# zwu88/TANTE

Measured on AMD Instinct MI355X. Metric: rollout frames/sec (fwd), TANTE on 256x256 Active Matter, higher is better.
Workload: dtype bf16

## Files before the change

tante_amd/_lib.py:

```python
import ctypes as C
import os

HERE = os.path.dirname(os.path.abspath(__file__))
LIB_PATH = os.environ.get("TANTE_LIB") or os.path.join(HERE, "lib", "libtante_hip.so")

F32, BF16 = 0, 1
ACT_NONE, ACT_GELU_ERF, ACT_GELU_TANH, ACT_RELU = 0, 1, 2, 3
A_LINEAR, A_PATCH_NHWC, A_PATCH_NCHW = 0, 1, 2
E_LINEAR, E_FILM, E_DECONV_NHWC, E_DECONV_NCHW = 0, 1, 2, 3
W_LINEAR, W_CONV_NHWC, W_DECONV_NHWC, W_DECONV_NCHW = 0, 1, 2, 3
W_LINEAR_T, W_CONV_NHWC_T, W_DECONV_NHWC_T, W_DECONV_NCHW_T = 4, 5, 6, 7

c_i32, c_i64, c_f32, c_vp = C.c_int32, C.c_int64, C.c_float, C.c_void_p


class PackGeom(C.Structure):
    _fields_ = [("n_pad", c_i32), ("k_pad", c_i32), ("nt", c_i32), ("cb", c_i32), ("bytes", c_i64)]


class Gemm(C.Structure):
    _fields_ = [
        ("a", c_vp), ("a_dtype", c_i32), ("a_mode", c_i32), ("M", c_i32), ("K", c_i32),
        ("a_s1", c_i64), ("a_s0", c_i64), ("a_off", c_i64), ("a_n0", c_i32),
        ("Hin", c_i32), ("Win", c_i32), ("Cin", c_i32), ("P", c_i32), ("ln", c_i32), ("ln_eps", c_f32),
# ... 195 lines not shown
    "tante_wgrad_multi": ([c_vp, c_vp, c_i32, c_i64, c_i32, c_i32, c_vp, c_vp, c_i32, c_i32, c_i32, c_i32, c_i32, c_i32, c_vp], c_i32),
    "tante_clip_value": ([c_vp, c_i64, c_f32, c_vp], c_i32),
    "tante_rt_reduce_bwd": ([c_vp, c_i32, c_i32, c_vp, c_vp], c_i32),
    "tante_last_error": ([], C.c_char_p),
    "tante_abi_version": ([], c_i32),
    "tante_set_option": ([C.c_char_p, c_i32], c_i32),
    "tante_nan_to_num": ([c_vp, c_vp, c_i64, c_vp], c_i32),
    "tante_head_fused_multi": ([c_i32, c_vp, c_vp, c_vp, c_i32, c_i64, c_i64, c_i64, c_i32, c_i32, c_i32, c_i32, c_i32, c_vp, c_i64, c_vp, c_i64,
                               c_vp], c_i32),
    "tante_head_fused_multi_streams": ([c_i32, c_vp, c_vp, c_vp, c_i32, c_i64, c_i64, c_i64, c_i32, c_i32, c_i32, c_i32, c_i32, c_vp, c_i64, c_vp, c_i64,
                               c_vp], c_i32),
    "tante_spectral_bf16out_supported": ([c_i64, c_i32, c_i32, c_i32, c_i32, c_i32, c_i32], c_i32),
    "tante_spectral_layer_bf16out": ([c_vp, c_i64, c_i32, c_i32, c_i32, c_vp, c_vp, c_i32, c_i32, c_i32, c_i32, c_vp, c_vp, c_i32, c_i32, c_vp, c_vp,
                                     c_i64, c_vp], c_i32),
    "tante_get_option": ([C.c_char_p, c_i32], c_i32),
    "tante_attention_masked": ([c_vp, c_vp, c_i32, c_i32, c_i32, c_i32, c_i32, c_i32, c_vp, c_i64, c_vp, c_vp], c_i32),
    "tante_attention_masked_bwd": ([c_vp, c_vp, c_vp, c_i32, c_i32, c_i32, c_i32, c_i32, c_i32, c_vp, c_i64, c_vp, c_vp, c_vp], c_i32),
    "tante_attention_flash_stats_floats": ([c_i32, C.POINTER(Seq)], c_i64),
    "tante_attention_flash_supported": ([c_i32, c_i32, c_i32, c_i32], c_i32),
    "tante_attention_flash": ([c_vp, c_vp, c_vp, c_i32, c_i32, c_i32, C.POINTER(Seq), c_i32, c_f32, C.c_uint64, c_vp], c_i32),
    "tante_attention_flash_bwd": ([c_vp, c_vp, c_vp, c_vp, c_vp, c_i32, c_i32, c_i32, C.POINTER(Seq), c_i32, c_f32, C.c_uint64, c_vp], c_i32),
    "tante_head_enc_supported": ([c_i32, c_i32], c_i32),
    "tante_head_enc_stream_bytes": ([c_i32], c_i64),
    "tante_head_enc_ws_bytes": ([c_i64], c_i64),
    "tante_pack_head_enc": ([c_vp] * 6 + [c_i32, c_i32, c_vp, c_vp], c_i32),
    "tante_head_enc_fused": ([c_i32, c_vp, c_vp, c_vp, c_i32, c_i64, c_i64, c_i64, c_i32, c_i32, c_i32, c_i32, c_i32, c_vp, c_i64, c_vp, c_i64,
                             c_vp, c_vp, c_vp, c_i64, c_vp], c_i32),
}

LIB_OPTIONS = ("TANTE_ATTN_BWD_HG", "TANTE_ATTN_BWD_NO_SPLIT", "TANTE_ATTN_BWD_VALU", "TANTE_ATTN_FWD_VALU", "TANTE_AXIS_BWD_SMALL_WGS",
               "TANTE_AXIS_BWD_WGS", "TANTE_AXIS_CT", "TANTE_AXIS_FILM", "TANTE_AXIS_GENERIC", "TANTE_AXIS_MFMA", "TANTE_AXIS_NT", "TANTE_AXIS_WGRAD_WGS",
               "TANTE_BLOCK_KERNEL", "TANTE_COLSUM_ROWS", "TANTE_CVIT_CHAIN_TOKENS", "TANTE_ENC23_SPLIT", "TANTE_FILM_BWD_ROWS",
               "TANTE_FS_GROUPS", "TANTE_FS_HALF", "TANTE_FS_SKEW", "TANTE_FS_WAVES", "TANTE_GEMM_NO_LITE", "TANTE_GEMM_SMALLM", "TANTE_GEMM_WGS", "TANTE_HEAD_WAVES",
               "TANTE_IM2COL_TILED", "TANTE_RESIZE_TILED", "TANTE_SPECTRAL_BF16OUT", "TANTE_SPECTRAL_DFT", "TANTE_SPECTRAL_X3", "TANTE_WGRAD_DEEP",
               "TANTE_WGRAD_JOBS", "TANTE_WGRAD_JOBS_WGS", "TANTE_WGRAD_NO_SLAB", "TANTE_WGRAD_NO_TR", "TANTE_WGRAD_REDUCE_NY",
               "TANTE_WGRAD_RG", "TANTE_WGRAD_SLAB_WGS", "TANTE_WGRAD_TR_WGS", "TANTE_WGRAD_WGS", "TANTE_XATTN_GPW", "TANTE_XATTN_VALU",)


_lib = None
ABI_VERSION = 14


def lib():
    global _lib
    if _lib is None:
        if not os.path.exists(LIB_PATH):
            raise RuntimeError(
                f"{LIB_PATH} is missing: build it with `python -m tante_amd.build` "
                "(or __graft_entry__.build()).  tante_amd has no CPU / eager fallback.")
        L = C.CDLL(LIB_PATH)
        for name, (argtypes, restype) in SIGNATURES.items():
            fn = getattr(L, name)
            fn.argtypes = argtypes
            fn.restype = restype
        got = int(L.tante_abi_version())
        if got != ABI_VERSION:
            raise RuntimeError(f"{LIB_PATH}: library ABI {got}, this binding expects {ABI_VERSION} -- a stale build (or a stale variant under "
                               "TANTE_LIB); rebuild with `python -m tante_amd.build`")
        _lib = L
        import warnings
        for k in LIB_OPTIONS:
            v = os.environ.get(k)
            if v is None:
                continue
            try:
                rc = L.tante_set_option(k.encode(), int(v))
            except ValueError:
# ... 20 lines not shown
```

tante_amd/csrc/block_sliced.hip:

```cpp
#include "common.hip.h"
#include "fused_common.hip.h"
#include "fs_common.hip.h"
#include "block_sliced.h"

#if (defined(FS_EXP_NO_SAVE) || defined(FS_EXP_LN_ID) || defined(FS_EXP_GELU_ID) || defined(FS_EXP_NO_RESID) || defined(FS_EXP_NO_STORE) || \
     defined(FS_EXP_TPROP_NO_STORE) || defined(FS_EXP_ROT) || defined(FS_EXP_NO_WLOAD) || defined(FS_EXP_MFMA32)) && !defined(TANTE_ABLATE)
#error "FS_EXP_* timing experiments produce wrong results on purpose: build them with -DTANTE_ABLATE (tools/build_variant.sh), never into the product library"
#endif

namespace {


struct FsArgs {
  float* x;
  const char* w;
  TanteSeq sq;
  int causal;
  float eps;
  int spw;
  unsigned magic;
  float* out;
  unsigned short *xh1, *qkv, *o, *xh2, *hpre, *act;
  float *st1, *x1, *st2;
  float p_drop;
// ... 50 lines not shown
}
__device__ __forceinline__ void tprop_apply(const TpropW& w, f32x4 (&xs)[4]) {
  f32x4 hid[4], yy[4];
#pragma unroll
  for (int e = 0; e < 4; ++e) {
    f32x4 h = w.b1v;
#pragma unroll
    for (int a = 0; a < 4; ++a) h = __builtin_amdgcn_mfma_f32_4x4x1f32(w.w1c[a], xs[a][e], h, 0, 0, 0);
    hid[e] = h;
  }
#pragma unroll
  for (int e = 0; e < 4; ++e) hid[e] = gelu_poly4<false>(hid[e]);
#pragma unroll
  for (int e = 0; e < 4; ++e) {
    f32x4 acc = f32x4{xs[0][e], xs[1][e], xs[2][e], xs[3][e]} + w.b2v;
#pragma unroll
    for (int j = 0; j < 4; ++j) acc = __builtin_amdgcn_mfma_f32_4x4x1f32(w.w2c[j], hid[e][j], acc, 0, 0, 0);
    yy[e] = acc;
  }
#pragma unroll
  for (int t = 0; t < 4; ++t) xs[t] = f32x4{yy[0][t], yy[1][t], yy[2][t], yy[3][t]};
}

constexpr int fs_group(int ntt, int nk) {
  int g = 1;
  for (int d = 1; d <= ntt; ++d)
    if (ntt % d == 0 && d * nk <= 8) g = d;
  return g;
}

template <int TPS, int NTT, int NW, bool TRAIN, int G = 1, bool TPROP = false, bool LASTQ = false>
__global__ __launch_bounds__(64 * NW * G, 2) void block_fs_kernel(FsArgs A) {
  static_assert(!TPROP || (TPS == 1 && !TRAIN), "the fused temporal propagator: T letter (L = 4), inference");
  static_assert(!LASTQ || (TPS == 1 && NW == 4 && G == 1 && !TRAIN), "the last-slot form: T letter (L = 4), 4 waves, inference");
  static_assert(G == 1 || (G == 2 && NW == 4), "the paired form is two 4-wave groups");
  constexpr int RT = 16 / NW;
  constexpr int HPW = RT / 2;
#ifndef FS_PF8
#define FS_PF8 3
#endif
#ifndef FS_PF4
#define FS_PF4 2
#endif
#ifdef FS_NO_TIGHT
  constexpr bool TIGHT = false;
#else
  constexpr bool TIGHT = (NW == 4 && NTT == 4 && (TRAIN || TPS == 0)) || (NW == 8 && NTT == 8);
#endif
  constexpr int PF = (NW == 8 ? FS_PF8 : FS_PF4) - (TIGHT ? 1 : 0);
  constexpr int IMG = 16 * NTT * FS_ROW;
  constexpr int LDS_G = 2 * IMG + 16 * NTT * NW * 8 + FS_BIAS_FLOATS * 4;
  extern __shared__ __attribute__((aligned(16))) char smem_all[];
  const int grp = G == 1 ? 0 : __builtin_amdgcn_readfirstlane((int)threadIdx.x >> 8);
  char* const smem = smem_all + grp * LDS_G;
  char* const bufA = smem;
  char* const bufB = smem + IMG;
  char* const stat = smem + 2 * IMG;
  float* const lbias = (float*)(stat + 16 * NTT * NW * 8);
  const int tid = threadIdx.x & (64 * NW - 1), lane = tid & 63, kk = lane >> 4, l15 = lane & 15;
  const int wave = __builtin_amdgcn_readfirstlane(tid >> 6);
#ifdef FS_XCD_SAMPLE
  const int vblock = (G == 1 && gridDim.x % 8 == 0) ? (int)((blockIdx.x & 7) * (gridDim.x >> 3) + (blockIdx.x >> 3)) : (int)blockIdx.x * G + grp;
#else
  const int vblock = (int)blockIdx.x * G + grp;
#endif
#ifndef FS_SKEW
#define FS_SKEW 1
#endif
  if constexpr (G == 2 && FS_SKEW) {
    if (grp == 1) __builtin_amdgcn_s_barrier();
  }
#ifdef FS_PRIO
  if constexpr (G == 1) {
    if ((__builtin_amdgcn_s_getreg(0x1804) & 1u) == (FS_PRIO & 1)) __builtin_amdgcn_s_setprio(3);
  }
#endif
  if constexpr (!TRAIN && G == 1) {
    if (A.skew > 0 && blockIdx.x >= (gridDim.x >> 1)) {
      for (int i = 0; i < A.skew; ++i) __builtin_amdgcn_s_sleep(8);
    }
  }
  float* const x = A.x;
  const unsigned long long smix = (TRAIN && A.seed_mix) ? *A.seed_mix : 0ull;
  const unsigned long long sd_attn = A.seed_attn ^ smix;
  const int L = A.sq.L;
  const int seq0 = vblock * A.spw;
  const int nlive = min(A.spw, A.sq.nseq - seq0) * L;
  const int nslot = A.spw * L;

  const FsW wq = fs_wstream(A.w, (unsigned)((RT * wave) * FS_FRAG + lane * 16));
  u32x4 wb[PF + 1][RT];
  FS_STAMP(0);
#ifdef TANTE_ABLATE
  if (A.stamps && lane == 0) {
    A.stamps[((long)vblock * 8 + wave) * 20 + 16] = __builtin_amdgcn_s_getreg((31 << 11) | 4);
    A.stamps[((long)vblock * 8 + wave) * 20 + 17] = __builtin_amdgcn_s_getreg((31 << 11) | 20);
    A.stamps[((long)vblock * 8 + wave) * 20 + 18] = __builtin_amdgcn_s_memrealtime();
  }
#endif
  int tslot[2];
  {
    const FsSeqMap smap(A.sq);
#pragma unroll
    for (int h = 0; h < (16 * NTT > 64 ? 2 : 1); ++h) {
      const int slot = lane + 64 * h;
      const int s = (int)(((unsigned)slot * A.magic) >> 16), p = slot - s * L;
      tslot[h] = slot < nlive ? (int)smap.token(A.sq, seq0 + s, p) : -1;
    }
  }
  auto tok_of = [&](int slot) { return __shfl(slot < 64 ? tslot[0] : tslot[16 * NTT > 64 ? 1 : 0], slot & 63); };
  for (int i = tid; i < FS_BIAS_FLOATS / 4; i += 64 * NW) *(f32x4*)(lbias + 4 * i) = *(const f32x4*)((const float*)(A.w + FS_W_BYTES) + 4 * i);
  FS_STAMP(1);
  int tokidx[NTT];
#pragma unroll
  for (int tt = 0; tt < NTT; ++tt) tokidx[tt] = tok_of(16 * tt + l15);

  constexpr int CPR = 4 * RT, RPI = 64 / CPR, ROWB = CPR * 16, TILEB = 16 * ROWB;
  constexpr int NSUB = (IMG / NW) / TILEB >= 2 ? 2 : 1;
  static_assert((IMG / NW) >= TILEB, "staging piece too small");
  char* const stg = bufA + wave * (IMG / NW);
  const int rrow = lane / CPR, rchunk = lane % CPR;
#ifdef FS_TPROP_RECOMPUTE
  auto srow = [&](int j) { return TPROP ? 4 * rrow + j : RPI * j + rrow; };
#else
  auto srow = [&](int j) { return RPI * j + rrow; };
#endif
  auto slice_load = [&](const float* __restrict__ src, f32x4 (&raw)[NTT][RT]) {
#pragma unroll
    for (int tt = 0; tt < NTT; ++tt)
#pragma unroll
      for (int j = 0; j < RT; ++j) {
        const int t = tok_of(16 * tt + srow(j));
        raw[tt][j] = *(const f32x4*)(src + (long)(t < 0 ? 0 : t) * FS_C + 16 * RT * wave + 4 * rchunk);
      }
  };
  auto slice_to_acc = [&](const f32x4 (&raw)[NTT][RT], f32x4 (&acc)[RT][NTT]) {
#pragma unroll
    for (int tt = 0; tt < NTT; ++tt) {
      char* sb = stg + (tt % NSUB) * TILEB;
#pragma unroll
      for (int j = 0; j < RT; ++j) {
        const int r = srow(j);
        *(f32x4*)(sb + r * ROWB + ((rchunk ^ (r & (CPR - 1))) << 4)) = raw[tt][j];
      }
#pragma unroll
      for (int rt = 0; rt < RT; ++rt) acc[rt][tt] = *(const f32x4*)(sb + l15 * ROWB + (((4 * rt + kk) ^ (l15 & (CPR - 1))) << 4));
    }
  };
  constexpr int CPB = 2 * RT, RPB = 64 / CPB;
  const int brow = lane / CPB, bchunk = lane % CPB;
  auto img_rows_store = [&](const char* img, int tt, unsigned short* __restrict__ dst, long dstride, int dcol) {
#pragma unroll
    for (int j = 0; j < 16 / RPB; ++j) {
      const int r = RPB * j + brow, t = tok_of(16 * tt + r);
      const u32x4 v = *(const u32x4*)(img + tt * 8192 + r * FS_ROW + (((CPB * wave + bchunk) ^ r) << 4));
#ifdef FS_EXP_NO_SAVE
      if (t >= 0 && v[0] == 0x12345u) *(u32x4*)(dst + (long)t * dstride + dcol + 16 * RT * wave + 8 * bchunk) = v;
#else
      if (t >= 0) *(u32x4*)(dst + (long)t * dstride + dcol + 16 * RT * wave + 8 * bchunk) = v;
#endif
    }
  };
  auto slice_store = [&](float* __restrict__ dst, const f32x4 (&acc)[RT][NTT]) {
#pragma unroll
    for (int tt = 0; tt < NTT; ++tt) {
      char* sb = stg + (tt % NSUB) * TILEB;
#pragma unroll
      for (int rt = 0; rt < RT; ++rt) *(f32x4*)(sb + l15 * ROWB + (((4 * rt + kk) ^ (l15 & (CPR - 1))) << 4)) = acc[rt][tt];
#pragma unroll
      for (int j = 0; j < RT; ++j) {
        const int r = RPI * j + rrow, t = tok_of(16 * tt + r);
        const f32x4 v = *(const f32x4*)(sb + r * ROWB + ((rchunk ^ (r & (CPR - 1))) << 4));
#ifdef FS_NT_STORE
        if (t >= 0) __builtin_nontemporal_store(v, (f32x4*)(dst + (long)t * FS_C + 16 * RT * wave + 4 * rchunk));
#else
        if (t >= 0 && (!LASTQ || (r & 3) == 3)) {
          if constexpr (TRAIN) *(f32x4*)(dst + (long)t * FS_C + 16 * RT * wave + 4 * rchunk) = v;
          else st_wt16(dst + (long)t * FS_C + 16 * RT * wave + 4 * rchunk, v);
        }
#endif
      }
    }
  };

  constexpr bool ln1_done = TPROP;
  if constexpr (TPROP) {
    {
      constexpr int GPW = 4 * NTT / NW;
      f32x4 xv[GPW][4];
#pragma unroll
      for (int i = 0; i < GPW; ++i)
#pragma unroll
        for (int t = 0; t < 4; ++t) {
          const int tk = tok_of(4 * (wave * GPW + i) + t);
          xv[i][t] = *(const f32x4*)(x + (long)(tk < 0 ? 0 : tk) * FS_C + 4 * lane);
        }
      fs_wring_prime<0, RT, PF>(wq, wb);
      TpropW tw;
      tprop_weights(A.tprop, lane, tw);
#pragma unroll
      for (int i = 0; i < GPW; ++i) {
        tprop_apply(tw, xv[i]);
#pragma unroll
        for (int t = 0; t < 4; ++t) {
          const f32x4 y = xv[i][t];
          const int tk = tok_of(4 * (wave * GPW + i) + t);
          const bool live = tk >= 0;
#ifndef FS_TPROP_RECOMPUTE
#ifndef FS_EXP_TPROP_NO_STORE
          if (live && (!LASTQ || t == 3)) *(f32x4*)(x + (long)tk * FS_C + 4 * lane) = y;
#endif
#endif
          float sm = (y[0] + y[1]) + (y[2] + y[3]);
          float sq = fmaf(y[0], y[0], fmaf(y[1], y[1], fmaf(y[2], y[2], y[3] * y[3])));
          sm = rows_sum(row16_sum(sm));
          sq = rows_sum(row16_sum(sq));
          const float mean = sm * (1.0f / FS_C);
          const float var = fmaxf(sq * (1.0f / FS_C) - mean * mean, 0.0f);
          const float rstd = live ? rsqrtf(var + A.eps) : 0.0f;
          const float sh = live ? -mean * rstd : 0.0f;
          const int slot = 4 * (wave * GPW + i) + t;
          u32x2 o2;
          o2[0] = pack_bf16x2(fmaf(y[0], rstd, sh), fmaf(y[1], rstd, sh));
          o2[1] = pack_bf16x2(fmaf(y[2], rstd, sh), fmaf(y[3], rstd, sh));
          *(u32x2*)(bufA + slot * FS_ROW + (((lane >> 1) ^ (slot & 15)) << 4) + (lane & 1) * 8) = o2;
        }
      }
    }
  }
  if constexpr (!ln1_done) {
    constexpr int GPW = 4 * NTT / NW;
    static_assert(GPW * NW == 4 * NTT, "token rows must split evenly over the waves");
    f32x4 v[GPW][4];
    bool lv[GPW];
    int tis[GPW];
#pragma unroll
    for (int i = 0; i < GPW; ++i) {
      const int ti = tis[i] = tok_of(4 * (wave * GPW + i) + kk);
      lv[i] = ti >= 0;
      const float* row = x + (long)(lv[i] ? ti : 0) * FS_C;
#pragma unroll
      for (int j = 0; j < 4; ++j) v[i][j] = *(const f32x4*)(row + 4 * (l15 + 16 * j));
    }
    fs_wring_prime<0, RT, PF>(wq, wb);
#pragma unroll
    for (int i = 0; i < GPW; ++i) {
      float s = 0.f, q = 0.f;
#pragma unroll
      for (int j = 0; j < 4; ++j)
#pragma unroll
        for (int e = 0; e < 4; ++e) {
          s += v[i][j][e];
          q = fmaf(v[i][j][e], v[i][j][e], q);
        }
      s = row16_sum(s);
      q = row16_sum(q);
      const float mean = s * (1.0f / FS_C);
      const float var = fmaxf(q * (1.0f / FS_C) - mean * mean, 0.0f);
      const float rstd = lv[i] ? rsqrtf(var + A.eps) : 0.0f;
      const float sh = lv[i] ? -mean * rstd : 0.0f;
      const int slot = 4 * (wave * GPW + i) + kk, t15 = slot & 15;
#pragma unroll
      for (int j = 0; j < 4; ++j) {
        u32x2 o2;
        o2[0] = pack_bf16x2(fmaf(v[i][j][0], rstd, sh), fmaf(v[i][j][1], rstd, sh));
        o2[1] = pack_bf16x2(fmaf(v[i][j][2], rstd, sh), fmaf(v[i][j][3], rstd, sh));
        const int chunk = (l15 >> 1) + 8 * j;
        *(u32x2*)(bufA + slot * FS_ROW + ((chunk ^ t15) << 4) + (l15 & 1) * 8) = o2;
        if constexpr (TRAIN) {
#ifdef FS_EXP_NO_SAVE
          if (lv[i] && o2[0] == 0x12345u) *(u32x2*)(A.xh1 + (long)tis[i] * FS_C + 4 * (l15 + 16 * j)) = o2;
#else
          if (lv[i]) *(u32x2*)(A.xh1 + (long)tis[i] * FS_C + 4 * (l15 + 16 * j)) = o2;
#endif
        }
      }
      if constexpr (TRAIN) {
        if (lv[i] && l15 == 0) *(float2*)(A.st1 + 2 * (long)tis[i]) = make_float2(mean, rstd);
      }
    }
  }

  int rdo[4];
#pragma unroll
  for (int j = 0; j < 4; ++j) rdo[j] = l15 * FS_ROW + ((((j ^ (l15 >> 2)) << 2) | (kk ^ (l15 & 3))) << 4);
  int wro[RT];
#pragma unroll
  for (int rt = 0; rt < RT; ++rt) wro[rt] = l15 * FS_ROW + (((2 * RT * wave + 2 * rt + (kk >> 1)) ^ l15) << 4) + (kk & 1) * 8;

  const float* const bias = lbias + 16 * RT * wave + 4 * kk;

  FS_STAMP(2);
  __syncthreads();
  FS_STAMP(3);

  const f32x4 zero4 = f32x4{0.f, 0.f, 0.f, 0.f};
  constexpr int NP = (NTT + 1) / 2;
  u32x4 qf[HPW][NTT], kf[HPW][NTT];
  u32x4 vtf[HPW][2][NP];
  {
    f32x4 aq[RT][NTT];
#pragma unroll
    for (int j = 0; j < RT; ++j) {
      const f32x4 bq = *(const f32x4*)(bias + 16 * j);
#pragma unroll
      for (int tt = 0; tt < NTT; ++tt) aq[j][tt] = bq;
    }
    fs_slice_gemm<0, 24, NTT, RT, false, PF>(wq, wb, bufA, rdo, aq);
#pragma unroll
    for (int hh = 0; hh < HPW; ++hh)
#pragma unroll
      for (int tt = 0; tt < NTT; ++tt) qf[hh][tt] = pack8(aq[2 * hh][tt], aq[2 * hh + 1][tt]);
    if (TRAIN && A.qkv) {
      const float unscale = 1.0f / (0.17677669529663687f * 1.44269504088896340736f);
#pragma unroll
      for (int tt = 0; tt < NTT; ++tt) {
#pragma unroll
        for (int j = 0; j < RT; ++j) {
          const f32x4 qv = aq[j][tt] * unscale;
          u32x2 u;
          u[0] = pack_bf16x2(qv[0], qv[1]); u[1] = pack_bf16x2(qv[2], qv[3]);
          *(u32x2*)(bufB + tt * 8192 + wro[j]) = u;
        }
        img_rows_store(bufB, tt, A.qkv, 3 * FS_C, 0);
      }
    }
  }
  FS_STAMP(4);
  {
    f32x4 ak[RT][NTT];
#pragma unroll
    for (int j = 0; j < RT; ++j) {
      const f32x4 bk = TRAIN ? *(const f32x4*)(bias + 1024 + 16 * j) : zero4;
#pragma unroll
      for (int tt = 0; tt < NTT; ++tt) ak[j][tt] = bk;
    }
    fs_slice_gemm<1, 24, NTT, RT, false, PF>(wq, wb, bufA, rdo, ak);
#pragma unroll
    for (int hh = 0; hh < HPW; ++hh)
#pragma unroll
      for (int tt = 0; tt < NTT; ++tt) kf[hh][tt] = pack8(ak[2 * hh][tt], ak[2 * hh + 1][tt]);
    if (TRAIN && A.qkv) {
#pragma unroll
      for (int tt = 0; tt < NTT; ++tt) {
#pragma unroll
        for (int j = 0; j < RT; ++j) {
          u32x2 u;
          u[0] = pack_bf16x2(ak[j][tt][0], ak[j][tt][1]); u[1] = pack_bf16x2(ak[j][tt][2], ak[j][tt][3]);
          *(u32x2*)(bufB + tt * 8192 + wro[j]) = u;
        }
        img_rows_store(bufB, tt, A.qkv, 3 * FS_C, FS_C);
      }
    }
  }
  FS_STAMP(5);
  {
    f32x4 av[RT][NTT];
#pragma unroll
    for (int j = 0; j < RT; ++j) {
      const float bv = TRAIN ? lbias[1280 + 16 * RT * wave + 16 * j + l15] : 0.0f;
#pragma unroll
      for (int tt = 0; tt < NTT; ++tt) av[j][tt] = f32x4{bv, bv, bv, bv};
    }
    fs_slice_gemm<2, 24, NTT, RT, true, PF>(wq, wb, bufA, rdo, av);
    if (TRAIN && A.qkv) {
#pragma unroll
      for (int tt = 0; tt < NTT; ++tt) {
#pragma unroll
        for (int r = 0; r < 4; ++r) {
          const int row = 4 * kk + r;
#pragma unroll
          for (int j = 0; j < RT; ++j) {
            const __bf16 b = (__bf16)av[j][tt][r];
            *(unsigned short*)(bufB + tt * 8192 + row * FS_ROW + (((CPB * wave + 2 * j + (l15 >> 3)) ^ row) << 4) + (l15 & 7) * 2) =
                __builtin_bit_cast(unsigned short, b);
          }
        }
        img_rows_store(bufB, tt, A.qkv, 3 * FS_C, 2 * FS_C);
      }
    }
#pragma unroll
    for (int hh = 0; hh < HPW; ++hh)
#pragma unroll
      for (int p = 0; p < NP; ++p)
#pragma unroll
        for (int dt = 0; dt < 2; ++dt)
          vtf[hh][dt][p] = (2 * p + 1 < NTT) ? pack8(av[2 * hh + dt][2 * p], av[2 * hh + dt][2 * p + 1]) : pack8(av[2 * hh + dt][2 * p], zero4);
  }
  FS_STAMP(6);
  if constexpr (G == 2 && FS_SKEW) __builtin_amdgcn_s_barrier();

  {
    unsigned allow1 = 0xfu;
    bool nomask = true;
    if constexpr (TPS == 1) {
      allow1 = 0u;
      const int si = (int)(((unsigned)l15 * A.magic) >> 16), pi = l15 - si * L;
#pragma unroll
      for (int r = 0; r < 4; ++r) {
        const int j = 4 * kk + r, sj = (int)(((unsigned)j * A.magic) >> 16), pj = j - sj * L;
        allow1 |= ((sj == si && (!A.causal || pj <= pi)) ? 1u : 0u) << r;
      }
      nomask = (L == 16) && !A.causal;
    }
    constexpr int NK = TPS > 0 ? TPS : NTT;
    constexpr int QG = fs_group(NTT, NK);
    static_for<HPW * (NTT / QG)>([&](auto hg_c) {
      constexpr int hh = decltype(hg_c)::value / (NTT / QG), q0 = (decltype(hg_c)::value % (NTT / QG)) * QG;
      f32x4 sc[QG][NK];
      unsigned allow[QG];
      float mx[QG], sum[QG];
      static_for<QG>([&](auto qt_c) {
        constexpr int q = decltype(qt_c)::value, qt = q0 + q;
        constexpr int k0 = TPS > 0 ? (qt / TPS) * TPS : 0;
#pragma unroll
        for (int j = 0; j < NK; ++j) sc[q][j] = mfma_bf16(kf[hh][k0 + j], qf[hh][qt], zero4);
      });
#pragma unroll
      for (int qt = 0; qt < QG; ++qt) {
        if constexpr (TPS == 0) {
          const int qs = 16 * (q0 + qt) + l15, si = (int)(((unsigned)qs * A.magic) >> 16), pi = qs - si * L;
          allow[qt] = 0u;
#pragma unroll
          for (int j = 0; j < NK; ++j)
#pragma unroll
// ... 88 lines not shown
        constexpr int k0 = TPS > 0 ? ((q0 + qt) / TPS) * TPS : 0;
        constexpr int g0 = k0 / 2, g1 = (k0 + NK - 1) / 2;
        o[qt][0] = o[qt][1] = zero4;
        static_for<g1 - g0 + 1>([&](auto g_c) {
          constexpr int g = g0 + decltype(g_c)::value;
          constexpr int ja = 2 * g - k0, jb = 2 * g + 1 - k0;
          f32x4 pa = zero4, pb = zero4;
          if constexpr (ja >= 0 && ja < NK) pa = sc[qt][ja];
          if constexpr (jb >= 0 && jb < NK) pb = sc[qt][jb];
          const u32x4 pf = pack8(pa, pb);
          o[qt][0] = mfma_bf16(vtf[hh][0][g], pf, o[qt][0]);
          o[qt][1] = mfma_bf16(vtf[hh][1][g], pf, o[qt][1]);
        });
      });
#pragma unroll
      for (int qt = 0; qt < QG; ++qt) {
        const float inv = sum[qt] > 0.0f ? __builtin_amdgcn_rcpf(sum[qt]) : 0.0f;
        const f32x4 o0 = o[qt][0] * inv, o1 = o[qt][1] * inv;
        u32x2 w0, w1;
        w0[0] = pack_bf16x2(o0[0], o0[1]); w0[1] = pack_bf16x2(o0[2], o0[3]);
        w1[0] = pack_bf16x2(o1[0], o1[1]); w1[1] = pack_bf16x2(o1[2], o1[3]);
        *(u32x2*)(bufB + (q0 + qt) * 8192 + wro[2 * hh]) = w0;
        *(u32x2*)(bufB + (q0 + qt) * 8192 + wro[2 * hh + 1]) = w1;
      }
    });
  }
  if constexpr (TRAIN) {
#pragma unroll
    for (int tt = 0; tt < NTT; ++tt) img_rows_store(bufB, tt, A.o, FS_C, 0);
  }

  FS_STAMP(7);
  asm volatile("" ::: "memory");
  f32x4 xraw[NTT][RT];
#ifndef FS_RESID_FIRST
  fs_wring_prime<3, RT, PF>(wq, wb);
#endif
#ifdef FS_EXP_NO_RESID
#pragma unroll
  for (int tt = 0; tt < NTT; ++tt)
#pragma unroll
    for (int j = 0; j < RT; ++j) xraw[tt][j] = f32x4{(float)tt, 1.f, 2.f, (float)j};
#else
  slice_load(x, xraw);
#endif
#ifdef FS_RESID_FIRST
  fs_wring_prime<3, RT, PF>(wq, wb);
#endif
  FS_STAMP(8);
  __syncthreads();
  FS_STAMP(9);

  f32x4 x1[RT][NTT];
#pragma unroll
  for (int rt = 0; rt < RT; ++rt) {
    const f32x4 bo = *(const f32x4*)(bias + (TRAIN ? 1536 : 256) + 16 * rt);
#pragma unroll
    for (int tt = 0; tt < NTT; ++tt) x1[rt][tt] = bo;
  }
  fs_slice_gemm<3, 48, NTT, RT, false, PF>(wq, wb, bufB, rdo, x1);
  auto drop_add = [&](f32x4 (&acc)[RT][NTT], f32x4 (&res)[RT][NTT], unsigned long long seed) {
    if constexpr (TRAIN) {
      if (A.p_drop > 0.0f) {
        const float ksc = 1.0f / (1.0f - A.p_drop);
#pragma unroll
        for (int tt = 0; tt < NTT; ++tt) {
          const unsigned long long i0 = (unsigned long long)(tokidx[tt] < 0 ? 0 : tokidx[tt]) * FS_C + 16 * RT * wave + 4 * kk;
#pragma unroll
          for (int rt = 0; rt < RT; ++rt) {
            const unsigned k01 = dropout_keep2(seed, i0 + 16 * rt, A.p_drop), k23 = dropout_keep2(seed, i0 + 16 * rt + 2, A.p_drop);
            acc[rt][tt][0] = (k01 & 1u) ? acc[rt][tt][0] * ksc : 0.0f;
            acc[rt][tt][1] = (k01 & 2u) ? acc[rt][tt][1] * ksc : 0.0f;
            acc[rt][tt][2] = (k23 & 1u) ? acc[rt][tt][2] * ksc : 0.0f;
            acc[rt][tt][3] = (k23 & 2u) ? acc[rt][tt][3] * ksc : 0.0f;
          }
        }
      }
    }
#pragma unroll
    for (int rt = 0; rt < RT; ++rt)
#pragma unroll
      for (int tt = 0; tt < NTT; ++tt) acc[rt][tt] += res[rt][tt];
  };
#ifdef FS_TPROP_RECOMPUTE
  if constexpr (TPROP) {
    static_assert(!TPROP || RT == 4, "a lane's row group = the four time steps of a sequence");
    TpropW tw;
    tprop_weights(A.tprop, lane, tw);
#pragma unroll
    for (int tt = 0; tt < NTT; ++tt) tprop_apply(tw, xraw[tt]);
  }
#endif
  {
    f32x4 xr[RT][NTT];
    slice_to_acc(xraw, xr);
    drop_add(x1, xr, A.seed_out ^ smix);
  }
  if constexpr (TRAIN) {
    if (A.x1) slice_store(A.x1, x1);
  }
  FS_STAMP(10);
#pragma unroll
  for (int tt = 0; tt < NTT; ++tt) {
    float s = 0.f, q = 0.f;
#pragma unroll
    for (int rt = 0; rt < RT; ++rt)
#pragma unroll
      for (int r = 0; r < 4; ++r) {
        s += x1[rt][tt][r];
        q = fmaf(x1[rt][tt][r], x1[rt][tt][r], q);
      }
    s = rows_sum(s);
    q = rows_sum(q);
    if (kk == 0) *(float2*)(stat + ((16 * tt + l15) * NW + wave) * 8) = make_float2(s, q);
  }
  __syncthreads();
  FS_STAMP(11);
#pragma unroll
  for (int tt = 0; tt < NTT; ++tt) {
    const f32x4* sp = (const f32x4*)(stat + (16 * tt + l15) * NW * 8);
    float s = 0.f, q = 0.f;
#pragma unroll
    for (int j = 0; j < NW / 2; ++j) {
      const f32x4 a = sp[j];
      s += a[0] + a[2];
      q += a[1] + a[3];
    }
    const float mean = s * (1.0f / FS_C);
    const float var = fmaxf(q * (1.0f / FS_C) - mean * mean, 0.0f);
    const float rstd = rsqrtf(var + A.eps);
    const float sh = -mean * rstd;
#pragma unroll
    for (int rt = 0; rt < RT; ++rt) {
      u32x2 o2;
#ifdef FS_EXP_LN_ID
      o2[0] = pack_bf16x2(x1[rt][tt][0], x1[rt][tt][1]);
      o2[1] = pack_bf16x2(x1[rt][tt][2], x1[rt][tt][3]);
#else
      o2[0] = pack_bf16x2(fmaf(x1[rt][tt][0], rstd, sh), fmaf(x1[rt][tt][1], rstd, sh));
      o2[1] = pack_bf16x2(fmaf(x1[rt][tt][2], rstd, sh), fmaf(x1[rt][tt][3], rstd, sh));
#endif
      *(u32x2*)(bufA + tt * 8192 + wro[rt]) = o2;
    }
    if constexpr (TRAIN) {
      img_rows_store(bufA, tt, A.xh2, FS_C, 0);
      if (wave == 0 && kk == 0 && tokidx[tt] >= 0) *(float2*)(A.st2 + 2 * (long)tokidx[tt]) = make_float2(mean, rstd);
    }
  }
  __syncthreads();
  FS_STAMP(12);

  {
    f32x4 h[RT][NTT];
#pragma unroll
    for (int rt = 0; rt < RT; ++rt) {
      const f32x4 b1 = *(const f32x4*)(bias + 512 + 16 * rt);
#pragma unroll
      for (int tt = 0; tt < NTT; ++tt) h[rt][tt] = b1;
    }
    fs_slice_gemm<4, 48, NTT, RT, false, PF>(wq, wb, bufA, rdo, h);
    FS_STAMP(13);
    if constexpr (G == 2 && FS_SKEW) __builtin_amdgcn_s_barrier();
#pragma unroll
    for (int tt = 0; tt < NTT; ++tt) {
      if constexpr (TRAIN) {
#pragma unroll
        for (int rt = 0; rt < RT; ++rt) {
          u32x2 hp;
          hp[0] = pack_bf16x2(h[rt][tt][0], h[rt][tt][1]);
          hp[1] = pack_bf16x2(h[rt][tt][2], h[rt][tt][3]);
          *(u32x2*)(bufB + tt * 8192 + wro[rt]) = hp;
        }
        img_rows_store(bufB, tt, A.hpre, FS_C, 0);
      }
#pragma unroll
      for (int rt = 0; rt < RT; ++rt) {
#ifdef FS_EXP_GELU_ID
        const f32x4 g = h[rt][tt];
#else
        const f32x4 g = gelu_poly4<true>(h[rt][tt]);
#endif
        u32x2 o2;
        o2[0] = pack_bf16x2(g[0], g[1]);
        o2[1] = pack_bf16x2(g[2], g[3]);
        *(u32x2*)(bufB + tt * 8192 + wro[rt]) = o2;
      }
      if constexpr (TRAIN) img_rows_store(bufB, tt, A.act, FS_C, 0);
    }
  }
  __syncthreads();
  FS_STAMP(14);

  {
    f32x4 y2[TRAIN ? RT : 1][TRAIN ? NTT : 1];
    if constexpr (TRAIN) {
#pragma unroll
      for (int rt = 0; rt < RT; ++rt) {
        const f32x4 b2 = *(const f32x4*)(bias + 768 + 16 * rt);
#pragma unroll
        for (int tt = 0; tt < NTT; ++tt) y2[rt][tt] = b2;
      }
      fs_slice_gemm<5, 48, NTT, RT, false, PF>(wq, wb, bufB, rdo, y2);
      drop_add(y2, x1, A.seed_mlp ^ smix);
#pragma unroll
      for (int rt = 0; rt < RT; ++rt)
#pragma unroll
        for (int tt = 0; tt < NTT; ++tt) x1[rt][tt] = y2[rt][tt];
    } else {
#pragma unroll
      for (int rt = 0; rt < RT; ++rt) {
        const f32x4 b2 = *(const f32x4*)(bias + 768 + 16 * rt);
#pragma unroll
        for (int tt = 0; tt < NTT; ++tt) x1[rt][tt] += b2;
      }
      fs_slice_gemm<5, 48, NTT, RT, false, PF>(wq, wb, bufB, rdo, x1);
    }
    FS_STAMP(15);
#ifdef TANTE_ABLATE
    if (A.stamps && lane == 0) A.stamps[((long)vblock * 8 + wave) * 20 + 19] = __builtin_amdgcn_s_memrealtime();
#endif
#ifdef FS_EXP_NO_STORE
#pragma unroll
    for (int tt = 0; tt < NTT; ++tt)
      if (tokidx[tt] >= 0) {
        float* row = (TRAIN ? A.out : x) + (long)tokidx[tt] * FS_C + 16 * RT * wave + 4 * kk;
        f32x4 sacc = x1[0][tt];
#pragma unroll
        for (int rt = 1; rt < RT; ++rt) sacc += x1[rt][tt];
        if (sacc[0] == 1.2345f) *(f32x4*)row = sacc;
      }
#else
    slice_store(TRAIN ? A.out : x, x1);
#endif
  }
  if constexpr (G == 2 && FS_SKEW) {
    if (grp == 0) __builtin_amdgcn_s_barrier();
  }
}

__device__ __forceinline__ void fs_pack_body(int bid, const float* __restrict__ w_in, const float* __restrict__ b_in, const float* __restrict__ g1,
                                             const float* __restrict__ be1, const float* __restrict__ w_out, const float* __restrict__ b_out,
                                             const float* __restrict__ w1, const float* __restrict__ b1, const float* __restrict__ g2,
                                             const float* __restrict__ be2, const float* __restrict__ w2, const float* __restrict__ b2,
                                             char* __restrict__ dst) {
  constexpr int C = FS_C;
  const float qscale = 0.17677669529663687f * 1.44269504088896340736f;
  const int nfrag = FS_W_BYTES / FS_FRAG;
  if (bid < nfrag / 4) {
    const int f = bid * 4 + (threadIdx.x >> 6), lane = threadIdx.x & 63, l15 = lane & 15, kk = lane >> 4;
    const int g = f % 16, ks = (f / 16) % 8, m = f / 128;
    const int row = (m < 3 ? m * C : 0) + 16 * g + l15;
    const float* src = m < 3 ? w_in : (m == 3 ? w_out : (m == 4 ? w1 : w2));
    const float* gamma = m < 3 ? g1 : (m == 4 ? g2 : nullptr);
    const float scale = m == 0 ? qscale : 1.0f;
    float v[8];
#pragma unroll
// ... 146 lines not shown
  A.out = nullptr;
  A.seed_mix = nullptr;
  A.tprop = tprop;
  if (tr) {
    if (sq.L > 64) return -4;
    A.out = tr->out; A.xh1 = (unsigned short*)tr->xh1; A.st1 = tr->st1; A.qkv = (unsigned short*)tr->qkv; A.o = (unsigned short*)tr->o;
    A.x1 = tr->x1; A.xh2 = (unsigned short*)tr->xh2; A.st2 = tr->st2; A.hpre = (unsigned short*)tr->hpre; A.act = (unsigned short*)tr->act;
    A.p_drop = tr->p_drop; A.seed_attn = tr->seed_attn; A.seed_out = tr->seed_out; A.seed_mlp = tr->seed_mlp;
    A.seed_mix = tante_seed_mix_ptr();
  }
  A.stamps = nullptr;
#ifdef TANTE_ABLATE
  A.stamps = g_fs_stamps;
#endif
  const int L = sq.L, nw = (tr || tprop || lastq) ? 4 : fs_waves(L);
  A.magic = (65536u + (unsigned)L - 1u) / (unsigned)L;
  int tps = 0;
  if (16 % L == 0) tps = 1;
  else if (!causal && (L == 32 || L == 48 || L == 64)) tps = L / 16;
  const int full = nw == 8 ? 8 : 4, tq = nw == 8 ? 6 : 3;
  const long resident = 256L * (8 / nw);
  auto rounds = [&](int ntt) {
    const int spw = 16 * ntt / L;
    const long nwg = (sq.nseq + spw - 1) / spw;
    return ((nwg + resident - 1) / resident) * ntt;
  };
  int ntt = full;
  if (tps == 3) ntt = tq;
  else if (tps >= 1 && (16 * tq) % L == 0 && (16 * tq) / L >= 1 && (tps == 1 || tq % tps == 0) && rounds(tq) < rounds(full)) ntt = tq;
  if (!tr && nw == 4 && (tps == 1 || tps == 2) && 32 % L == 0 && tante_opt("TANTE_FS_HALF", 1)) {
    const int spw_full = 16 * ntt / L;
    if (((long)sq.nseq + spw_full - 1) / spw_full * 4 <= resident) ntt = 2;
  }
  if (lastq && ntt == tq) ntt = full;
  A.spw = tps ? 16 * ntt / L : (16 * full) / L;
  const int nwg = (sq.nseq + A.spw - 1) / A.spw;
  A.skew = (!tr && nw == 4 && nwg > 256 && nwg <= 512) ? tante_opt("TANTE_FS_SKEW", 0) : 0;
  if (lastq) {
    if (ntt == 2) fs_launch_last<2>(A, nwg, s);
    else fs_launch_last<4>(A, nwg, s);
    return 0;
  }
  const int key = nw * 100 + tps * 10 + ntt;
  switch (key) {
    case 412:
      if (A.tprop) fs_launch_tt<1, 2, 4, false, 1, true>(A, nwg, s);
      else fs_launch_tt<1, 2, 4, false>(A, nwg, s);
      break;
    case 422: fs_launch_tt<2, 2, 4, false>(A, nwg, s); break;
    case 818: fs_launch_t<1, 8, 8>(A, nwg, s); break;
    case 816: fs_launch_t<1, 6, 8>(A, nwg, s); break;
    case 828: fs_launch_t<2, 8, 8>(A, nwg, s); break;
    case 826: fs_launch_t<2, 6, 8>(A, nwg, s); break;
    case 836: fs_launch_t<3, 6, 8>(A, nwg, s); break;
    case 848: fs_launch_t<4, 8, 8>(A, nwg, s); break;
    case 808: fs_launch_t<0, 8, 8>(A, nwg, s); break;
    case 414: fs_launch_t<1, 4, 4>(A, nwg, s); break;
    case 413: fs_launch_t<1, 3, 4>(A, nwg, s); break;
    case 424: fs_launch_t<2, 4, 4>(A, nwg, s); break;
    case 433: fs_launch_t<3, 3, 4>(A, nwg, s); break;
    case 444: fs_launch_t<4, 4, 4>(A, nwg, s); break;
    case 404: fs_launch_t<0, 4, 4>(A, nwg, s); break;
    default: return -3;
  }
  return 0;
}
```

Before: 18860.

## Compute only last-slot query tokens in the last-query fused block kernel

In the last-query (LASTQ) form of the fused transformer block, only every fourth token slot (the last time step) is needed. The Q projection, attention, output projection, LayerNorm and MLP now run on a compacted set of query tiles (NQT = NTT/4 rounded up) instead of all NTT tiles, while K and V are still computed for every slot. A separate weight ring buffer with deeper prefetch handles the narrower GEMMs, and an option to force the tile count is added. This cuts MFMA and LDS work in the later stages, at the cost of more complex indexing and extra register use for the second weight ring.

New measurement: 18920 (median of 6 runs). Within noise of the previous version (+0.3%).

```diff
diff --git a/tante_amd/_lib.py b/tante_amd/_lib.py
--- a/tante_amd/_lib.py
+++ b/tante_amd/_lib.py
@@ -251,7 +251,7 @@
                "TANTE_AXIS_BWD_WGS", "TANTE_AXIS_CT", "TANTE_AXIS_FILM", "TANTE_AXIS_GENERIC", "TANTE_AXIS_MFMA", "TANTE_AXIS_NT", "TANTE_AXIS_WGRAD_WGS",
                "TANTE_BLOCK_KERNEL", "TANTE_COLSUM_ROWS", "TANTE_CVIT_CHAIN_TOKENS", "TANTE_ENC23_SPLIT", "TANTE_FILM_BWD_ROWS",
                "TANTE_FS_GROUPS", "TANTE_FS_HALF", "TANTE_FS_SKEW", "TANTE_FS_WAVES", "TANTE_GEMM_NO_LITE", "TANTE_GEMM_SMALLM", "TANTE_GEMM_WGS", "TANTE_HEAD_WAVES",
-               "TANTE_IM2COL_TILED", "TANTE_RESIZE_TILED", "TANTE_SPECTRAL_BF16OUT", "TANTE_SPECTRAL_DFT", "TANTE_SPECTRAL_X3", "TANTE_WGRAD_DEEP",
+               "TANTE_IM2COL_TILED", "TANTE_LAST_TILES", "TANTE_RESIZE_TILED", "TANTE_SPECTRAL_BF16OUT", "TANTE_SPECTRAL_DFT", "TANTE_SPECTRAL_X3", "TANTE_WGRAD_DEEP",
                "TANTE_WGRAD_JOBS", "TANTE_WGRAD_JOBS_WGS", "TANTE_WGRAD_NO_SLAB", "TANTE_WGRAD_NO_TR", "TANTE_WGRAD_REDUCE_NY",
                "TANTE_WGRAD_RG", "TANTE_WGRAD_SLAB_WGS", "TANTE_WGRAD_TR_WGS", "TANTE_WGRAD_WGS", "TANTE_XATTN_GPW", "TANTE_XATTN_VALU",)
 
diff --git a/tante_amd/csrc/block_sliced.hip b/tante_amd/csrc/block_sliced.hip
--- a/tante_amd/csrc/block_sliced.hip
+++ b/tante_amd/csrc/block_sliced.hip
@@ -106,7 +106,8 @@
 template <int TPS, int NTT, int NW, bool TRAIN, int G = 1, bool TPROP = false, bool LASTQ = false>
 __global__ __launch_bounds__(64 * NW * G, 2) void block_fs_kernel(FsArgs A) {
   static_assert(!TPROP || (TPS == 1 && !TRAIN), "the fused temporal propagator: T letter (L = 4), inference");
-  static_assert(!LASTQ || (TPS == 1 && NW == 4 && G == 1 && !TRAIN), "the last-slot form: T letter (L = 4), 4 waves, inference");
+  static_assert(!LASTQ || (TPS == 1 && NW == 4 && G == 1 && !TRAIN && (NTT == 2 || NTT == 4)), "the last-slot form: T letter (L = 4), 4 waves, inference");
+  constexpr int NQT = LASTQ ? (NTT + 3) / 4 : NTT;
   static_assert(G == 1 || (G == 2 && NW == 4), "the paired form is two 4-wave groups");
   constexpr int RT = 16 / NW;
   constexpr int HPW = RT / 2;
@@ -122,6 +123,7 @@
   constexpr bool TIGHT = (NW == 4 && NTT == 4 && (TRAIN || TPS == 0)) || (NW == 8 && NTT == 8);
 #endif
   constexpr int PF = (NW == 8 ? FS_PF8 : FS_PF4) - (TIGHT ? 1 : 0);
+  constexpr int PFQ = LASTQ ? 5 : PF;
   constexpr int IMG = 16 * NTT * FS_ROW;
   constexpr int LDS_G = 2 * IMG + 16 * NTT * NW * 8 + FS_BIAS_FLOATS * 4;
   extern __shared__ __attribute__((aligned(16))) char smem_all[];
@@ -164,6 +166,8 @@
 
   const FsW wq = fs_wstream(A.w, (unsigned)((RT * wave) * FS_FRAG + lane * 16));
   u32x4 wb[PF + 1][RT];
+  u32x4 wbq_[LASTQ ? PFQ + 1 : 1][RT];
+  auto& wbq = [&]() -> auto& { if constexpr (LASTQ) return wbq_; else return wb; }();
   FS_STAMP(0);
 #ifdef TANTE_ABLATE
   if (A.stamps && lane == 0) {
@@ -199,18 +203,19 @@
 #else
   auto srow = [&](int j) { return RPI * j + rrow; };
 #endif
-  auto slice_load = [&](const float* __restrict__ src, f32x4 (&raw)[NTT][RT]) {
-#pragma unroll
-    for (int tt = 0; tt < NTT; ++tt)
+  auto qslot = [&](int tt, int r) { return LASTQ ? 64 * tt + 4 * r + 3 : 16 * tt + r; };
+  auto slice_load = [&](const float* __restrict__ src, f32x4 (&raw)[NQT][RT]) {
+#pragma unroll
+    for (int tt = 0; tt < NQT; ++tt)
 #pragma unroll
       for (int j = 0; j < RT; ++j) {
-        const int t = tok_of(16 * tt + srow(j));
+        const int t = tok_of(qslot(tt, srow(j)));
         raw[tt][j] = *(const f32x4*)(src + (long)(t < 0 ? 0 : t) * FS_C + 16 * RT * wave + 4 * rchunk);
       }
   };
-  auto slice_to_acc = [&](const f32x4 (&raw)[NTT][RT], f32x4 (&acc)[RT][NTT]) {
-#pragma unroll
-    for (int tt = 0; tt < NTT; ++tt) {
+  auto slice_to_acc = [&](const f32x4 (&raw)[NQT][RT], f32x4 (&acc)[RT][NQT]) {
+#pragma unroll
+    for (int tt = 0; tt < NQT; ++tt) {
       char* sb = stg + (tt % NSUB) * TILEB;
 #pragma unroll
       for (int j = 0; j < RT; ++j) {
@@ -235,20 +240,20 @@
 #endif
     }
   };
-  auto slice_store = [&](float* __restrict__ dst, const f32x4 (&acc)[RT][NTT]) {
-#pragma unroll
-    for (int tt = 0; tt < NTT; ++tt) {
+  auto slice_store = [&](float* __restrict__ dst, const f32x4 (&acc)[RT][NQT]) {
+#pragma unroll
+    for (int tt = 0; tt < NQT; ++tt) {
       char* sb = stg + (tt % NSUB) * TILEB;
 #pragma unroll
       for (int rt = 0; rt < RT; ++rt) *(f32x4*)(sb + l15 * ROWB + (((4 * rt + kk) ^ (l15 & (CPR - 1))) << 4)) = acc[rt][tt];
 #pragma unroll
       for (int j = 0; j < RT; ++j) {
-        const int r = RPI * j + rrow, t = tok_of(16 * tt + r);
+        const int r = RPI * j + rrow, t = tok_of(qslot(tt, r));
         const f32x4 v = *(const f32x4*)(sb + r * ROWB + ((rchunk ^ (r & (CPR - 1))) << 4));
 #ifdef FS_NT_STORE
         if (t >= 0) __builtin_nontemporal_store(v, (f32x4*)(dst + (long)t * FS_C + 16 * RT * wave + 4 * rchunk));
 #else
-        if (t >= 0 && (!LASTQ || (r & 3) == 3)) {
+        if (t >= 0) {
           if constexpr (TRAIN) *(f32x4*)(dst + (long)t * FS_C + 16 * RT * wave + 4 * rchunk) = v;
           else st_wt16(dst + (long)t * FS_C + 16 * RT * wave + 4 * rchunk, v);
         }
@@ -269,7 +274,8 @@
           const int tk = tok_of(4 * (wave * GPW + i) + t);
           xv[i][t] = *(const f32x4*)(x + (long)(tk < 0 ? 0 : tk) * FS_C + 4 * lane);
         }
-      fs_wring_prime<0, RT, PF>(wq, wb);
+      fs_wring_prime<LASTQ ? 1 : 0, RT, PF>(wq, wb);
+      if constexpr (LASTQ) fs_wring_prime<0, RT, PFQ>(wq, wbq);
       TpropW tw;
       tprop_weights(A.tprop, lane, tw);
 #pragma unroll
@@ -316,7 +322,8 @@
 #pragma unroll
       for (int j = 0; j < 4; ++j) v[i][j] = *(const f32x4*)(row + 4 * (l15 + 16 * j));
     }
-    fs_wring_prime<0, RT, PF>(wq, wb);
+    fs_wring_prime<LASTQ ? 1 : 0, RT, PF>(wq, wb);
+    if constexpr (LASTQ) fs_wring_prime<0, RT, PFQ>(wq, wbq);
 #pragma unroll
     for (int i = 0; i < GPW; ++i) {
       float s = 0.f, q = 0.f;
@@ -370,9 +377,9 @@
 
   const f32x4 zero4 = f32x4{0.f, 0.f, 0.f, 0.f};
   constexpr int NP = (NTT + 1) / 2;
-  u32x4 qf[HPW][NTT], kf[HPW][NTT];
+  u32x4 qf[HPW][NQT], kf[HPW][NTT];
   u32x4 vtf[HPW][2][NP];
-  {
+  if constexpr (!LASTQ) {
     f32x4 aq[RT][NTT];
 #pragma unroll
     for (int j = 0; j < RT; ++j) {
@@ -400,6 +407,24 @@
       }
     }
   }
+  if constexpr (LASTQ) {
+    const int qrow = (4 * l15 + 3) & (16 * NTT - 1);
+    int rdq[4];
+#pragma unroll
+    for (int j = 0; j < 4; ++j) rdq[j] = qrow * FS_ROW + ((((j ^ ((qrow >> 2) & 3)) << 2) | (kk ^ (qrow & 3))) << 4);
+    f32x4 aq[RT][NQT];
+#pragma unroll
+    for (int j = 0; j < RT; ++j) {
+      const f32x4 bq = *(const f32x4*)(bias + 16 * j);
+#pragma unroll
+      for (int tt = 0; tt < NQT; ++tt) aq[j][tt] = bq;
+    }
+    fs_slice_gemm<0, 8, NQT, RT, false, PFQ>(wq, wbq, bufA, rdq, aq);
+#pragma unroll
+    for (int hh = 0; hh < HPW; ++hh)
+#pragma unroll
+      for (int tt = 0; tt < NQT; ++tt) qf[hh][tt] = pack8(aq[2 * hh][tt], aq[2 * hh + 1][tt]);
+  }
   FS_STAMP(4);
   {
     f32x4 ak[RT][NTT];
@@ -461,10 +486,63 @@
         for (int dt = 0; dt < 2; ++dt)
           vtf[hh][dt][p] = (2 * p + 1 < NTT) ? pack8(av[2 * hh + dt][2 * p], av[2 * hh + dt][2 * p + 1]) : pack8(av[2 * hh + dt][2 * p], zero4);
   }
+  if constexpr (LASTQ) fs_wring_prime<3, RT, PFQ>(wq, wbq);
   FS_STAMP(6);
   if constexpr (G == 2 && FS_SKEW) __builtin_amdgcn_s_barrier();
 
-  {
+  if constexpr (LASTQ) {
+    constexpr int NKQ = NTT < 4 ? NTT : 4;
+    const bool mine = kk == (l15 & 3);
+    static_for<HPW>([&](auto h_c) {
+      constexpr int hh = decltype(h_c)::value;
+      f32x4 sc[NQT][NKQ];
+      float mx[NQT], sum[NQT];
+#pragma unroll
+      for (int qt = 0; qt < NQT; ++qt)
+#pragma unroll
+        for (int j = 0; j < NKQ; ++j) sc[qt][j] = mfma_bf16(kf[hh][NKQ * qt + j], qf[hh][qt], zero4);
+#pragma unroll
+      for (int qt = 0; qt < NQT; ++qt) {
+        float m = -INFINITY;
+#pragma unroll
+        for (int j = 0; j < NKQ; ++j)
+#pragma unroll
+          for (int r = 0; r < 4; ++r)
+            if (mine && (l15 >> 2) == j) m = fmaxf(m, sc[qt][j][r]);
+        mx[qt] = rows_max(m);
+      }
+#pragma unroll
+      for (int qt = 0; qt < NQT; ++qt) {
+        float sm = 0.0f;
+#pragma unroll
+        for (int j = 0; j < NKQ; ++j)
+#pragma unroll
+          for (int r = 0; r < 4; ++r) {
+            sc[qt][j][r] = (mine && (l15 >> 2) == j) ? __builtin_amdgcn_exp2f(sc[qt][j][r] - mx[qt]) : 0.0f;
+            sm += sc[qt][j][r];
+          }
+        sum[qt] = rows_sum(sm);
+      }
+#pragma unroll
+      for (int qt = 0; qt < NQT; ++qt) {
+        f32x4 o0 = zero4, o1 = zero4;
+#pragma unroll
+        for (int g = 0; g < NKQ / 2; ++g) {
+          const u32x4 pf = pack8(sc[qt][2 * g], sc[qt][2 * g + 1]);
+          o0 = mfma_bf16(vtf[hh][0][(NKQ / 2) * qt + g], pf, o0);
+          o1 = mfma_bf16(vtf[hh][1][(NKQ / 2) * qt + g], pf, o1);
+        }
+        const float inv = sum[qt] > 0.0f ? __builtin_amdgcn_rcpf(sum[qt]) : 0.0f;
+        o0 = o0 * inv;
+        o1 = o1 * inv;
+        u32x2 w0, w1;
+        w0[0] = pack_bf16x2(o0[0], o0[1]); w0[1] = pack_bf16x2(o0[2], o0[3]);
+        w1[0] = pack_bf16x2(o1[0], o1[1]); w1[1] = pack_bf16x2(o1[2], o1[3]);
+        *(u32x2*)(bufB + qt * 8192 + wro[2 * hh]) = w0;
+        *(u32x2*)(bufB + qt * 8192 + wro[2 * hh + 1]) = w1;
+      }
+    });
+  } else {
     unsigned allow1 = 0xfu;
     bool nomask = true;
     if constexpr (TPS == 1) {
@@ -619,39 +697,39 @@
 
   FS_STAMP(7);
   asm volatile("" ::: "memory");
-  f32x4 xraw[NTT][RT];
+  f32x4 xraw[NQT][RT];
 #ifndef FS_RESID_FIRST
-  fs_wring_prime<3, RT, PF>(wq, wb);
+  if constexpr (!LASTQ) fs_wring_prime<3, RT, PF>(wq, wb);
 #endif
 #ifdef FS_EXP_NO_RESID
 #pragma unroll
-  for (int tt = 0; tt < NTT; ++tt)
+  for (int tt = 0; tt < NQT; ++tt)
 #pragma unroll
     for (int j = 0; j < RT; ++j) xraw[tt][j] = f32x4{(float)tt, 1.f, 2.f, (float)j};
 #else
   slice_load(x, xraw);
 #endif
 #ifdef FS_RESID_FIRST
-  fs_wring_prime<3, RT, PF>(wq, wb);
+  if constexpr (!LASTQ) fs_wring_prime<3, RT, PF>(wq, wb);
 #endif
   FS_STAMP(8);
   __syncthreads();
   FS_STAMP(9);
 
-  f32x4 x1[RT][NTT];
+  f32x4 x1[RT][NQT];
 #pragma unroll
   for (int rt = 0; rt < RT; ++rt) {
     const f32x4 bo = *(const f32x4*)(bias + (TRAIN ? 1536 : 256) + 16 * rt);
 #pragma unroll
-    for (int tt = 0; tt < NTT; ++tt) x1[rt][tt] = bo;
-  }
-  fs_slice_gemm<3, 48, NTT, RT, false, PF>(wq, wb, bufB, rdo, x1);
-  auto drop_add = [&](f32x4 (&acc)[RT][NTT], f32x4 (&res)[RT][NTT], unsigned long long seed) {
+    for (int tt = 0; tt < NQT; ++tt) x1[rt][tt] = bo;
+  }
+  fs_slice_gemm<3, 48, NQT, RT, false, PFQ>(wq, wbq, bufB, rdo, x1);
+  auto drop_add = [&](f32x4 (&acc)[RT][NQT], f32x4 (&res)[RT][NQT], unsigned long long seed) {
     if constexpr (TRAIN) {
       if (A.p_drop > 0.0f) {
         const float ksc = 1.0f / (1.0f - A.p_drop);
 #pragma unroll
-        for (int tt = 0; tt < NTT; ++tt) {
+        for (int tt = 0; tt < NQT; ++tt) {
           const unsigned long long i0 = (unsigned long long)(tokidx[tt] < 0 ? 0 : tokidx[tt]) * FS_C + 16 * RT * wave + 4 * kk;
 #pragma unroll
           for (int rt = 0; rt < RT; ++rt) {
@@ -667,7 +745,7 @@
 #pragma unroll
     for (int rt = 0; rt < RT; ++rt)
 #pragma unroll
-      for (int tt = 0; tt < NTT; ++tt) acc[rt][tt] += res[rt][tt];
+      for (int tt = 0; tt < NQT; ++tt) acc[rt][tt] += res[rt][tt];
   };
 #ifdef FS_TPROP_RECOMPUTE
   if constexpr (TPROP) {
@@ -675,11 +753,11 @@
     TpropW tw;
     tprop_weights(A.tprop, lane, tw);
 #pragma unroll
-    for (int tt = 0; tt < NTT; ++tt) tprop_apply(tw, xraw[tt]);
+    for (int tt = 0; tt < NQT; ++tt) tprop_apply(tw, xraw[tt]);
   }
 #endif
   {
-    f32x4 xr[RT][NTT];
+    f32x4 xr[RT][NQT];
     slice_to_acc(xraw, xr);
     drop_add(x1, xr, A.seed_out ^ smix);
   }
@@ -688,7 +766,7 @@
   }
   FS_STAMP(10);
 #pragma unroll
-  for (int tt = 0; tt < NTT; ++tt) {
+  for (int tt = 0; tt < NQT; ++tt) {
     float s = 0.f, q = 0.f;
 #pragma unroll
     for (int rt = 0; rt < RT; ++rt)
@@ -704,7 +782,7 @@
   __syncthreads();
   FS_STAMP(11);
 #pragma unroll
-  for (int tt = 0; tt < NTT; ++tt) {
+  for (int tt = 0; tt < NQT; ++tt) {
     const f32x4* sp = (const f32x4*)(stat + (16 * tt + l15) * NW * 8);
     float s = 0.f, q = 0.f;
 #pragma unroll
@@ -738,18 +816,18 @@
   FS_STAMP(12);
 
   {
-    f32x4 h[RT][NTT];
+    f32x4 h[RT][NQT];
 #pragma unroll
     for (int rt = 0; rt < RT; ++rt) {
       const f32x4 b1 = *(const f32x4*)(bias + 512 + 16 * rt);
 #pragma unroll
-      for (int tt = 0; tt < NTT; ++tt) h[rt][tt] = b1;
-    }
-    fs_slice_gemm<4, 48, NTT, RT, false, PF>(wq, wb, bufA, rdo, h);
+      for (int tt = 0; tt < NQT; ++tt) h[rt][tt] = b1;
+    }
+    fs_slice_gemm<4, 48, NQT, RT, false, PFQ>(wq, wbq, bufA, rdo, h);
     FS_STAMP(13);
     if constexpr (G == 2 && FS_SKEW) __builtin_amdgcn_s_barrier();
 #pragma unroll
-    for (int tt = 0; tt < NTT; ++tt) {
+    for (int tt = 0; tt < NQT; ++tt) {
       if constexpr (TRAIN) {
 #pragma unroll
         for (int rt = 0; rt < RT; ++rt) {
@@ -779,28 +857,28 @@
   FS_STAMP(14);
 
   {
-    f32x4 y2[TRAIN ? RT : 1][TRAIN ? NTT : 1];
+    f32x4 y2[TRAIN ? RT : 1][TRAIN ? NQT : 1];
     if constexpr (TRAIN) {
 #pragma unroll
       for (int rt = 0; rt < RT; ++rt) {
         const f32x4 b2 = *(const f32x4*)(bias + 768 + 16 * rt);
 #pragma unroll
-        for (int tt = 0; tt < NTT; ++tt) y2[rt][tt] = b2;
-      }
-      fs_slice_gemm<5, 48, NTT, RT, false, PF>(wq, wb, bufB, rdo, y2);
+        for (int tt = 0; tt < NQT; ++tt) y2[rt][tt] = b2;
+      }
+      fs_slice_gemm<5, 48, NQT, RT, false, PFQ>(wq, wbq, bufB, rdo, y2);
       drop_add(y2, x1, A.seed_mlp ^ smix);
 #pragma unroll
       for (int rt = 0; rt < RT; ++rt)
 #pragma unroll
-        for (int tt = 0; tt < NTT; ++tt) x1[rt][tt] = y2[rt][tt];
+        for (int tt = 0; tt < NQT; ++tt) x1[rt][tt] = y2[rt][tt];
     } else {
 #pragma unroll
       for (int rt = 0; rt < RT; ++rt) {
         const f32x4 b2 = *(const f32x4*)(bias + 768 + 16 * rt);
 #pragma unroll
-        for (int tt = 0; tt < NTT; ++tt) x1[rt][tt] += b2;
-      }
-      fs_slice_gemm<5, 48, NTT, RT, false, PF>(wq, wb, bufB, rdo, x1);
+        for (int tt = 0; tt < NQT; ++tt) x1[rt][tt] += b2;
+      }
+      fs_slice_gemm<5, 48, NQT, RT, false, PFQ>(wq, wbq, bufB, rdo, x1);
     }
     FS_STAMP(15);
 #ifdef TANTE_ABLATE
@@ -808,7 +886,7 @@
 #endif
 #ifdef FS_EXP_NO_STORE
 #pragma unroll
-    for (int tt = 0; tt < NTT; ++tt)
+    for (int tt = 0; tt < NQT; ++tt)
       if (tokidx[tt] >= 0) {
         float* row = (TRAIN ? A.out : x) + (long)tokidx[tt] * FS_C + 16 * RT * wave + 4 * kk;
         f32x4 sacc = x1[0][tt];
@@ -1021,7 +1099,10 @@
     const int spw_full = 16 * ntt / L;
     if (((long)sq.nseq + spw_full - 1) / spw_full * 4 <= resident) ntt = 2;
   }
-  if (lastq && ntt == tq) ntt = full;
+  if (lastq) {
+    const int force = tante_opt("TANTE_LAST_TILES", 0);
+    ntt = (force == 2 || force == 4) ? force : (ntt == 2 ? 2 : 4);
+  }
   A.spw = tps ? 16 * ntt / L : (16 * full) / L;
   const int nwg = (sq.nseq + A.spw - 1) / A.spw;
   A.skew = (!tr && nw == 4 && nwg > 256 && nwg <= 512) ? tante_opt("TANTE_FS_SKEW", 0) : 0;
```
